# johndpope/SPEAK-hack

Hardware: NVIDIA B200
Metric: irfd_train_pairs_per_sec_256 (higher is better)
Workload: dtype bf16

## Files before the change

include/irfd_b200.h:

```cpp
#ifndef IRFD_B200_H_
#define IRFD_B200_H_

#include <stddef.h>
#include <stdint.h>

#ifdef __cplusplus
extern "C" {
#endif

#define IRFD_ABI_VERSION 1

#define IRFD_OK 0
#define IRFD_ERR_INVALID_ARGUMENT (-1)
#define IRFD_ERR_CUDA (-2)

typedef struct CUstream_st* irfd_stream_t;

int irfd_abi_version(void);
const char* irfd_last_error(void);

int irfd_conv_gemm_m_tiles(int n, int h, int w);
int irfd_conv_gemm_geometry(int n, int h, int w, int ksize, int wgroups, int* out_host);
int irfd_conv_gemm(const void* x, int n, int h, int w, int cin, const void* wk, int cout, int ksize, void* out,
                   void* out2, int mode, const float* bias, const float* nw, const float* noise, const float* sp1,
// ... 61 lines not shown
int irfd_conv_gemm_bnbwd_grouped(const void* x, int n, int h, int w, int cin, const void* wk, int cout, int ksize,
                                 void* out, const void* bn_z, const float* bn_mean, const float* bn_rstd,
                                 const float* const* bn_gamma, const float* const* bn_beta, float* partial,
                                 int stat_groups, int wgroups, int force_block_n, irfd_stream_t stream);
int irfd_conv_gemm_bnbwd_res_grouped(const void* x, int n, int h, int w, int cin, const void* wk, int cout, int ksize,
                                     void* out, const void* bn_z, const float* bn_mean, const float* bn_rstd,
                                     const void* g2, const void* mask_bits, float* partial, int stat_groups,
                                     int wgroups, int force_block_n, irfd_stream_t stream);
int irfd_bn_backward_finish_sets(const void* g, const void* z, const float* mean, const float* rstd,
                                 const float* const* gamma, void* dz, float* const* dgamma, float* const* dbeta,
                                 float grad_beta, int batch_stats, long long rows, int c, int groups, int nsets,
                                 const float* partial, int tiles, void* workspace, long long workspace_bytes,
                                 irfd_stream_t stream);

int irfd_pack_conv_weight(const float* w, void* dst, int o, int i, int taps, int mode, int kpad, irfd_stream_t stream);
int irfd_im2col_stem(const float* x, void* col, int n, int h, int w, int kpad, irfd_stream_t stream);
int irfd_im2col_3x3s2(const void* a, void* col, int n, int h, int w, int c, irfd_stream_t stream);
int irfd_col2im_3x3s2(const void* dcol, void* dx, int n, int h, int w, int c, irfd_stream_t stream);
int irfd_subsample2(const void* a, void* out, int n, int h, int w, int c, irfd_stream_t stream);
int irfd_scatter_add_s2(const void* a, const void* b, void* out, int n, int h, int w, int c, irfd_stream_t stream);
int irfd_maxpool_fwd(const void* a, void* out, void* argmax, int n, int h, int w, int c, irfd_stream_t stream);
int irfd_maxpool_bwd(const void* dout, const void* dout2, const void* argmax, void* dx, int n, int h, int w, int c,
                     irfd_stream_t stream);
int irfd_avgpool_fwd(const void* a, float* out, int n, int hw, int c, irfd_stream_t stream);
int irfd_avgpool_bwd(const float* dfeat, void* g, int n, int hw, int c, irfd_stream_t stream);
int irfd_nchw_to_nhwc_bf16(const float* in, void* out, int b, int c, int hw, int c_pad, irfd_stream_t stream);
int irfd_nhwc_bf16_to_nchw(const void* in, float* out, int b, int c, int hw, int c_pad, irfd_stream_t stream);

int irfd_const_input_fwd(const float* cst, const float* bias, const float* nw, const float* noise, const float* sp1,
                         const float* s1, void* a0, void* y0, int b, int c, irfd_stream_t stream);
int irfd_const_input_bwd(const void* dy, const void* a0, const float* noise, const float* sp1, float* dsp1, float* ds1,
                         float* dconst, float* dbias, float* dnw, int b, int c, irfd_stream_t stream);
int irfd_upsample2x_fwd(const void* in, void* out, int b, int h, int w, int c, irfd_stream_t stream);
int irfd_upsample2x_split_fwd(const void* in, const void* in_lo, void* out, int b, int h, int w, int c,
                              irfd_stream_t stream);
int irfd_const_input_split_fwd(const float* cst, const float* bias, const float* nw, const float* noise,
                               const float* sp1, const float* s1, void* a0, void* y0, void* y0_lo, int b, int c,
                               irfd_stream_t stream);
int irfd_upsample2x_bwd(const void* dout, void* din, int b, int h, int w, int c, irfd_stream_t stream);
int irfd_apply_noise_nchw(const float* x, const float* w, const float* noise, float* out, int b, int c, int hw,
                          irfd_stream_t stream);
int irfd_apply_style_nchw(const float* x, const float* style, float* out, int b, int c, int hw, irfd_stream_t stream);
long long irfd_style_bwd_workspace_bytes(int b, int hw, int c);
int irfd_style_bwd(const void* dy, const void* a, const float* noise, const float* sp1, void* dz, float* ds1,
                   float* dsp1, float* dbias, float* dnw, int b, int hw, int c, void* workspace,
                   long long workspace_bytes, irfd_stream_t stream);
// ... 49 lines not shown
```

speak_hack_b200/csrc/bn.cu:

```cuda
#include "host_util.h"
#include "rowvec.cuh"

namespace irfd {

constexpr int kMaxGroups = 4;
constexpr int kMaxSets = 4;
struct FSet {
  const float* p[kMaxSets];
};
struct FSetM {
  float* p[kMaxSets];
};
constexpr int kFinCh = 8;
constexpr int kFinLanes = 64;
constexpr int kFinThreads = kFinCh * kFinLanes;
constexpr int kFinWarps = kFinThreads / 32;
constexpr int kFinBatch = 8;

__device__ __forceinline__ void fin_partial_sums(const float* __restrict__ p0, const float* __restrict__ p1, size_t stride0,
                                                 size_t stride1, int n, int lane, double& a, double& b) {
  a = 0.0;
  b = 0.0;
  for (int t = lane; t < n; t += kFinLanes * kFinBatch) {
    float x[kFinBatch], y[kFinBatch];
#pragma unroll
    for (int u = 0; u < kFinBatch; ++u) {
      const int tt = t + u * kFinLanes;
      x[u] = tt < n ? __ldg(p0 + (size_t)tt * stride0) : 0.f;
      y[u] = tt < n ? __ldg(p1 + (size_t)tt * stride1) : 0.f;
    }
#pragma unroll
    for (int u = 0; u < kFinBatch; ++u) {
// ... 465 lines not shown
        L.g1, L.g2, L.act, L.z, L.mean, L.rstd, L.gamma, L.beta, L.partial, L.g_out, L.grows, L.c, L.rpb, L.gps,
        zigzag());
  else
    bn_bwd_reduce_kernel<HAS_G2, MASK, false><<<L.grid, kRvThreads, L.smem, L.stream>>>(
        L.g1, L.g2, L.act, L.z, L.mean, L.rstd, L.gamma, L.beta, L.partial, nullptr, L.grows, L.c, L.rpb, L.gps,
        zigzag());
  bn_bwd_finalize_kernel<<<dim3(L.c / kFinCh, L.nsets), kFinThreads, 0, L.stream>>>(L.partial, L.nblk, L.c, (double)L.grows,
                                                                             L.dgamma, L.dbeta, L.grad_beta, L.c1, L.c2,
                                                                             L.batch_stats, L.gps);
  if (L.g_out != nullptr)
    bn_bwd_apply_kernel<false, 0, false><<<L.grid, kRvThreads, 0, L.stream>>>(
        L.g_out, nullptr, nullptr, L.z, L.mean, L.rstd, L.gamma, L.beta, L.c1, L.c2, L.dz, nullptr, L.grows, L.c, L.rpb,
        L.gps);
  else
    bn_bwd_apply_kernel<HAS_G2, MASK, false><<<L.grid, kRvThreads, 0, L.stream>>>(
        L.g1, L.g2, L.act, L.z, L.mean, L.rstd, L.gamma, L.beta, L.c1, L.c2, L.dz, nullptr, L.grows, L.c, L.rpb,
        L.gps);
}

}

using namespace irfd;

static FSet make_fset(const float* const* ptrs, int nsets) {
  FSet f;
  for (int i = 0; i < kMaxSets; ++i) f.p[i] = (ptrs != nullptr && i < nsets) ? ptrs[i] : nullptr;
  return f;
}
static FSetM make_fsetm(float* const* ptrs, int nsets) {
  FSetM f;
  for (int i = 0; i < kMaxSets; ++i) f.p[i] = (ptrs != nullptr && i < nsets) ? ptrs[i] : nullptr;
  return f;
}

extern "C" int irfd_bn_finalize_sets(const float* psum, const float* psq, int tiles, int c, long long count, float eps,
                                     float momentum, float* mean, float* rstd, float* const* running_mean,
                                     float* const* running_var, int running_updates, int groups, int nsets,
                                     cudaStream_t stream) {
  IRFD_CHECK_ARG(psum && psq && mean && rstd && tiles > 0 && c > 0 && count > 0, "bn_finalize: bad argument");
  IRFD_CHECK_ARG(groups >= 1 && groups <= kMaxGroups, "bn_finalize: 1..4 statistic groups per set");
  IRFD_CHECK_ARG(nsets >= 1 && nsets <= kMaxSets, "bn_finalize: 1..4 parameter sets");
  IRFD_CHECK_ARG(c % kFinCh == 0, "bn_finalize: C must be a multiple of 8 (got %d)", c);
  IRFD_CHECK_ARG((running_mean == nullptr) == (running_var == nullptr), "bn_finalize: running buffers come in pairs");
  bn_finalize_kernel<<<dim3(c / kFinCh, nsets), kFinThreads, 0, stream>>>(psum, psq, tiles, c, (double)count, eps, momentum,
                                                                     mean, rstd, make_fsetm(running_mean, nsets),
                                                                     make_fsetm(running_var, nsets), running_updates,
                                                                     groups);
  IRFD_CHECK_LAUNCH();
  return IRFD_OK;
}

// ... 198 lines not shown
```

speak_hack_b200/csrc/layout.cu:

```cuda
#include "host_util.h"
#include "rowvec.cuh"

namespace irfd {

__global__ void pack_weight_kernel(const float* __restrict__ w, __nv_bfloat16* __restrict__ dst, int O, int I, int T,
                                   int mode, int kpad) {
  const size_t idx = (size_t)blockIdx.x * blockDim.x + threadIdx.x;
  if (mode == 3) {
    if (idx >= (size_t)O * kpad) return;
    const int o = idx / kpad, k = idx % kpad;
    dst[idx] = __float2bfloat16(k < I * T ? w[(size_t)o * I * T + k] : 0.f);
    return;
  }
  if (idx >= (size_t)O * I * T) return;
  const int tap = idx % T;
  const int i = (idx / T) % I;
  const int o = idx / ((size_t)T * I);
  const __nv_bfloat16 v = __float2bfloat16(w[idx]);
  size_t d;
  if (mode == 0) d = ((size_t)o * T + tap) * I + i;
  else if (mode == 1) d = ((size_t)i * T + (T - 1 - tap)) * O + o;
  else d = ((size_t)tap * I + i) * O + o;
  dst[d] = v;
}
// ... 44 lines not shown
#pragma unroll
    for (int t = 0; t < 8; ++t) f[t] = off[t] >= 0 ? srow[off[t] + 2 * ow] : 0.f;
    store8(col + (pix0 + ow) * kpad + v * 8, f);
  }
}

__global__ void im2col_3x3s2_kernel(const __nv_bfloat16* __restrict__ a, __nv_bfloat16* __restrict__ col, int N, int H,
                                    int W, int C) {
  const unsigned Ho = (H + 1) / 2, Wo = (W + 1) / 2, vc = C / 8;
  const unsigned idx = blockIdx.x * blockDim.x + threadIdx.x;
  const size_t total = (size_t)N * Ho * Wo * 9 * vc;
  if (idx >= total) return;
  const int v = idx % vc;
  const int tap = (idx / vc) % 9;
  const unsigned pix = idx / (vc * 9u);
  const int ow = pix % Wo, oh = (pix / Wo) % Ho, n = pix / ((unsigned)Wo * Ho);
  const int ih = oh * 2 + tap / 3 - 1, iw = ow * 2 + tap % 3 - 1;
  uint4 val = make_uint4(0, 0, 0, 0);
  if (ih >= 0 && ih < H && iw >= 0 && iw < W)
    val = *reinterpret_cast<const uint4*>(a + (((size_t)n * H + ih) * W + iw) * C + v * 8);
  *reinterpret_cast<uint4*>(col + ((size_t)pix * 9 + tap) * C + v * 8) = val;
}

__global__ void col2im_3x3s2_kernel(const __nv_bfloat16* __restrict__ dcol, __nv_bfloat16* __restrict__ dx, int N,
                                    int H, int W, int C) {
  const unsigned Ho = H / 2, Wo = W / 2, vc = C / 8;
  const unsigned idx = blockIdx.x * blockDim.x + threadIdx.x;
  const size_t total = (size_t)N * H * W * vc;
  if (idx >= total) return;
  const int v = idx % vc;
  const unsigned pix = idx / vc;
  const int w = pix % W, h = (pix / W) % H, n = pix / ((unsigned)W * H);
  float acc[8];
#pragma unroll
  for (int t = 0; t < 8; ++t) acc[t] = 0.f;
  for (int kh = 0; kh < 3; ++kh) {
    const int th = h - kh + 1;
    if (th < 0 || (th & 1)) continue;
    const int oh = th >> 1;
    if (oh >= Ho) continue;
    for (int kw = 0; kw < 3; ++kw) {
      const int tw = w - kw + 1;
      if (tw < 0 || (tw & 1)) continue;
      const int ow = tw >> 1;
      if (ow >= Wo) continue;
      float f[8];
// ... 20 lines not shown
__global__ void scatter_add_s2_kernel(const __nv_bfloat16* __restrict__ a, const __nv_bfloat16* __restrict__ b,
                                      __nv_bfloat16* __restrict__ out, int N, int H, int W, int C) {
  const unsigned vc = C / 8;
  const unsigned idx = blockIdx.x * blockDim.x + threadIdx.x;
  if (idx >= (size_t)N * H * W * vc) return;
  const int v = idx % vc;
  const unsigned pix = idx / vc;
  const int w = pix % W, h = (pix / W) % H, n = pix / ((unsigned)W * H);
  float f[8];
  if (a != nullptr) load8(a + (size_t)pix * C + v * 8, f);
  else {
#pragma unroll
    for (int t = 0; t < 8; ++t) f[t] = 0.f;
  }
  if (!(h & 1) && !(w & 1)) {
    float g[8];
    load8(b + (((size_t)n * (H / 2) + h / 2) * (W / 2) + w / 2) * C + v * 8, g);
#pragma unroll
    for (int t = 0; t < 8; ++t) f[t] += g[t];
  }
  store8(out + (size_t)pix * C + v * 8, f);
}

__global__ void maxpool_fwd_kernel(const __nv_bfloat16* __restrict__ a, __nv_bfloat16* __restrict__ out,
                                   uint8_t* __restrict__ arg, int N, int H, int W, int C) {
  const unsigned Ho = (H + 1) / 2, Wo = (W + 1) / 2, vc = C / 8;
  const unsigned idx = blockIdx.x * blockDim.x + threadIdx.x;
  if (idx >= (size_t)N * Ho * Wo * vc) return;
  const int v = idx % vc;
  const unsigned pix = idx / vc;
  const int ow = pix % Wo, oh = (pix / Wo) % Ho, n = pix / ((unsigned)Wo * Ho);
  float best[8];
  int bi[8];
#pragma unroll
  for (int t = 0; t < 8; ++t) {
    best[t] = -INFINITY;
    bi[t] = 0;
  }
  for (int tap = 0; tap < 9; ++tap) {
    const int ih = oh * 2 + tap / 3 - 1, iw = ow * 2 + tap % 3 - 1;
    if (ih < 0 || ih >= H || iw < 0 || iw >= W) continue;
    float f[8];
    load8(a + (((size_t)n * H + ih) * W + iw) * C + v * 8, f);
#pragma unroll
    for (int t = 0; t < 8; ++t)
      if (f[t] > best[t]) {
        best[t] = f[t];
        bi[t] = tap;
      }
  }
  store8(out + (size_t)pix * C + v * 8, best);
  uint2 packed;
  packed.x = bi[0] | (bi[1] << 8) | (bi[2] << 16) | (bi[3] << 24);
  packed.y = bi[4] | (bi[5] << 8) | (bi[6] << 16) | (bi[7] << 24);
  *reinterpret_cast<uint2*>(arg + (size_t)pix * C + v * 8) = packed;
}

__global__ void __launch_bounds__(256)
maxpool_bwd_kernel(const __nv_bfloat16* __restrict__ dout, const __nv_bfloat16* __restrict__ dout2,
                   const uint8_t* __restrict__ arg, __nv_bfloat16* __restrict__ dx, int N, int H, int W, int C) {
  const unsigned Ho = H / 2, Wo = W / 2, vc = C >> 3;
  const unsigned q = blockIdx.y * blockDim.x + threadIdx.x;
  if (q >= Wo * vc) return;
  const int j = q / vc, v = q - j * vc;
  const int n = blockIdx.x / Ho, i = blockIdx.x - n * Ho;
  float g[2][2][8];
  uint2 am[2][2];
#pragma unroll
  for (int a = 0; a < 2; ++a)
#pragma unroll
    for (int b = 0; b < 2; ++b) {
      am[a][b] = make_uint2(0xffffffffu, 0xffffffffu);
#pragma unroll
      for (int t = 0; t < 8; ++t) g[a][b][t] = 0.f;
      if ((unsigned)(i + a) < Ho && (unsigned)(j + b) < Wo) {
        const size_t op = (((size_t)n * Ho + i + a) * Wo + j + b) * C + v * 8;
        am[a][b] = __ldg(reinterpret_cast<const uint2*>(arg + op));
        unpack8(ldg16(dout + op), g[a][b]);
// ... 119 lines not shown
  return IRFD_OK;
}

extern "C" int irfd_im2col_stem(const float* x, void* col, int n, int h, int w, int kpad, cudaStream_t stream) {
  IRFD_CHECK_ARG(x && col && kpad >= 152 && kpad % 8 == 0 && h > 0 && w > 0, "im2col_stem: bad argument");
  const size_t smem = (size_t)21 * (w + 6) * sizeof(float);
  IRFD_CHECK_ARG(n > 0 && smem <= 48 * 1024, "im2col_stem: image too wide for the row stage (W <= 579, got %d)", w);
  IRFD_CHECK_ARG(kStemPixPar * (kpad / 8) <= 256 && (kpad / 8) % 4 == 0, "im2col_stem: kpad a multiple of 32 and <= 256");
  im2col_stem_kernel<<<(unsigned)(n * ((h + 1) / 2)), kStemPixPar * (kpad / 8), smem, stream>>>(x, BF(col), n, h, w,
                                                                                              kpad);
  IRFD_CHECK_LAUNCH();
  return IRFD_OK;
}

extern "C" int irfd_im2col_3x3s2(const void* a, void* col, int n, int h, int w, int c, cudaStream_t stream) {
  IRFD_CHECK_ARG(a && col && c % 8 == 0 && h > 0 && w > 0, "im2col_3x3s2: bad argument");
  const size_t total = (size_t)n * ((h + 1) / 2) * ((w + 1) / 2) * 9 * (c / 8);
  CHECK_TOTAL32(total);
  im2col_3x3s2_kernel<<<GRID1D(total)>>>(CBF(a), BF(col), n, h, w, c);
  IRFD_CHECK_LAUNCH();
  return IRFD_OK;
}

extern "C" int irfd_col2im_3x3s2(const void* dcol, void* dx, int n, int h, int w, int c, cudaStream_t stream) {
  IRFD_CHECK_ARG(dcol && dx && c % 8 == 0 && h % 2 == 0 && w % 2 == 0, "col2im_3x3s2: bad argument");
  const size_t total = (size_t)n * h * w * (c / 8);
  CHECK_TOTAL32(total);
  col2im_3x3s2_kernel<<<GRID1D(total)>>>(CBF(dcol), BF(dx), n, h, w, c);
  IRFD_CHECK_LAUNCH();
  return IRFD_OK;
}

extern "C" int irfd_subsample2(const void* a, void* out, int n, int h, int w, int c, cudaStream_t stream) {
  IRFD_CHECK_ARG(a && out && c % 8 == 0 && h > 0 && w > 0, "subsample2: bad argument");
  const size_t total = (size_t)n * ((h + 1) / 2) * ((w + 1) / 2) * (c / 8);
  CHECK_TOTAL32(total);
  subsample2_kernel<<<GRID1D(total)>>>(CBF(a), BF(out), n, h, w, c);
  IRFD_CHECK_LAUNCH();
  return IRFD_OK;
}

extern "C" int irfd_scatter_add_s2(const void* a, const void* b, void* out, int n, int h, int w, int c,
                                   cudaStream_t stream) {
  IRFD_CHECK_ARG(b && out && c % 8 == 0 && h % 2 == 0 && w % 2 == 0, "scatter_add_s2: bad argument");
  const size_t total = (size_t)n * h * w * (c / 8);
  CHECK_TOTAL32(total);
  scatter_add_s2_kernel<<<GRID1D(total)>>>(CBF(a), CBF(b), BF(out), n, h, w, c);
  IRFD_CHECK_LAUNCH();
  return IRFD_OK;
}

extern "C" int irfd_maxpool_fwd(const void* a, void* out, void* argmax, int n, int h, int w, int c,
                                cudaStream_t stream) {
  IRFD_CHECK_ARG(a && out && argmax && c % 8 == 0 && h > 0 && w > 0, "maxpool_fwd: bad argument");
  const size_t total = (size_t)n * ((h + 1) / 2) * ((w + 1) / 2) * (c / 8);
  CHECK_TOTAL32(total);
  maxpool_fwd_kernel<<<GRID1D(total)>>>(CBF(a), BF(out), reinterpret_cast<uint8_t*>(argmax), n, h, w, c);
  IRFD_CHECK_LAUNCH();
  return IRFD_OK;
}

extern "C" int irfd_maxpool_bwd(const void* dout, const void* dout2, const void* argmax, void* dx, int n, int h, int w,
                                int c, cudaStream_t stream) {
  IRFD_CHECK_ARG(dout && dx && argmax && c % 8 == 0 && h % 2 == 0 && w % 2 == 0, "maxpool_bwd: bad argument");
  IRFD_CHECK_ARG((long long)w * c < (1ll << 24) && (long long)n * h < (1ll << 31), "maxpool_bwd: bad shape");
  maxpool_bwd_kernel<<<dim3((unsigned)(n * (h / 2)), (unsigned)(((w / 2) * (c / 8) + 255) / 256)), 256, 0, stream>>>(
      CBF(dout), CBF(dout2), reinterpret_cast<const uint8_t*>(argmax), BF(dx), n, h, w, c);
  IRFD_CHECK_LAUNCH();
  return IRFD_OK;
}

extern "C" int irfd_avgpool_fwd(const void* a, float* out, int n, int hw, int c, cudaStream_t stream) {
  IRFD_CHECK_ARG(a && out && c % 8 == 0 && c <= 2048 && hw > 0, "avgpool_fwd: bad argument");
  avgpool_fwd_kernel<<<n, kRvThreads, 2048 * sizeof(float), stream>>>(CBF(a), out, hw, c);
  IRFD_CHECK_LAUNCH();
  return IRFD_OK;
}

extern "C" int irfd_avgpool_bwd(const float* dfeat, void* g, int n, int hw, int c, cudaStream_t stream) {
  IRFD_CHECK_ARG(dfeat && g && c % 8 == 0 && hw > 0, "avgpool_bwd: bad argument");
// ... 23 lines not shown
```

speak_hack_b200/csrc/rowvec.cuh:

```cuda
#pragma once
#include <stdlib.h>
#include "ptx.cuh"

namespace irfd {

constexpr int kRvThreads = 256;

struct RowVec {
  int cv;
  int row_lane;
  int rows_par;
  bool active;
  __device__ RowVec(int C) {
    const int vec_per_row = C >> 3;
    rows_par = kRvThreads / vec_per_row;
    if (rows_par < 1) rows_par = 1;
    cv = threadIdx.x % vec_per_row;
    row_lane = threadIdx.x / vec_per_row;
    active = row_lane < rows_par;
  }
};

constexpr int kRowBatch = 4;

__device__ __forceinline__ uint4 ldg16(const __nv_bfloat16* p) { return __ldg(reinterpret_cast<const uint4*>(p)); }
__device__ __forceinline__ void unpack8(const uint4& u, float (&f)[8]) {
  float2 a = unpack_bf16x2(u.x), b = unpack_bf16x2(u.y), c = unpack_bf16x2(u.z), d = unpack_bf16x2(u.w);
  f[0] = a.x; f[1] = a.y; f[2] = b.x; f[3] = b.y; f[4] = c.x; f[5] = c.y; f[6] = d.x; f[7] = d.y;
}
__device__ __forceinline__ void load8(const __nv_bfloat16* p, float (&f)[8]) {
  const uint4 u = *reinterpret_cast<const uint4*>(p);
  unpack8(u, f);
}
__device__ __forceinline__ void store8(__nv_bfloat16* p, const float (&f)[8]) {
  uint4 u;
  u.x = pack_bf16x2(f[0], f[1]);
  u.y = pack_bf16x2(f[2], f[3]);
  u.z = pack_bf16x2(f[4], f[5]);
  u.w = pack_bf16x2(f[6], f[7]);
  *reinterpret_cast<uint4*>(p) = u;
}
__device__ __forceinline__ void loadf8(const float* p, float (&f)[8]) {
  const float4 a = *reinterpret_cast<const float4*>(p);
  const float4 b = *reinterpret_cast<const float4*>(p + 4);
  f[0] = a.x; f[1] = a.y; f[2] = a.z; f[3] = a.w; f[4] = b.x; f[5] = b.y; f[6] = b.z; f[7] = b.w;
}

template <int K>
__device__ __forceinline__ void block_reduce_rows(const RowVec& rv, int C, float (&acc)[K][8], float* smem, float* dst,
                                                  size_t dst_stride) {
  if (rv.active) {
#pragma unroll
    for (int k = 0; k < K; ++k)
#pragma unroll
      for (int t = 0; t < 8; ++t) smem[((size_t)k * rv.rows_par + rv.row_lane) * C + rv.cv * 8 + t] = acc[k][t];
  }
  __syncthreads();
  if (rv.active && rv.row_lane == 0) {
#pragma unroll
    for (int k = 0; k < K; ++k)
#pragma unroll
      for (int t = 0; t < 8; ++t) {
        float s = 0.f;
        for (int l = 0; l < rv.rows_par; ++l) s += smem[((size_t)k * rv.rows_par + l) * C + rv.cv * 8 + t];
        dst[k * dst_stride + rv.cv * 8 + t] = s;
      }
  }
}

inline int row_block_waves() {
// ... 21 lines not shown
```

speak_hack_b200/encoder_group.py:

```python
from __future__ import annotations

import os
from typing import Dict, List, Optional

import torch
import torch.nn as nn

from . import ops
from .encoder import BN_EPS, BN_MOMENTUM, MAX_STEM_W, MIN_HW, ResNet50Encoder, trainable_shape


fold_bn_reduce = os.environ.get("IRFD_BN_FOLD", "1") != "0"
fold_bn3_reduce = os.environ.get("IRFD_BN3_FOLD", "0") != "0"


def _stack_pack(convs, mode, kpad=0):
    return ops.pack_conv_weights_stacked([c.weight for c in convs], mode, kpad)


class _Stats:
    __slots__ = ("mean", "rstd")

    def __init__(self, mean, rstd):
        self.mean, self.rstd = mean, rstd


def _group_inference(grp: "EncoderGroup", x, col0=None):
    encs = grp.encoders
    E = len(encs)
    x = x.contiguous().to(torch.float32)
    n, _, h, w = x.shape
    if col0 is None:
        col0 = ops.im2col_stem(x, 192)
    sc, sh = ops.bn_eval_affine_sets([e[1] for e in encs])
    a0 = ops.conv_gemm_affine_grouped(col0, _stack_pack([e[0] for e in encs], ops.PACK_FLAT, 192), 1, sc, sh, relu=True,
                                      wgroups=E, a_shared=True).view(E * n, ops.half_up(h), ops.half_up(w), 64)
# ... 28 lines not shown


class _EncoderGroupFn(torch.autograd.Function):

    @staticmethod
    def forward(ctx, x, grp, stat_groups, col0, recorded, *params):
        encs: List[ResNet50Encoder] = grp.encoders
        E = len(encs)
        G = stat_groups
        GT = E * G
        U = 2 if (recorded and all(getattr(e, "_recompute_bn_update", False) for e in encs)) else 1
        x = x.contiguous().to(torch.float32)
        n, _, h, w = x.shape

        def stats(bns, s, q, rows_total):
            mean, rstd = ops.bn_finalize_sets(s, q, rows_total // GT, BN_EPS, BN_MOMENTUM,
                                              [b.running_mean for b in bns], [b.running_var for b in bns], U, G, E)
            return _Stats(mean, rstd)

        def apply(z, st, bns, relu=True, res=None, bn2=None, want_mask=False):
            return ops.bn_apply_sets(z, st.mean, st.rstd, [b.weight for b in bns], [b.bias for b in bns], res=res,
                                     bn2=bn2, relu=relu, groups=GT, want_mask=want_mask)

        S = {}
        if col0 is None:
            col0 = ops.im2col_stem(x, 192)
        bn0 = [e[1] for e in encs]
        z0, s, q = ops.conv_gemm_grouped(col0, _stack_pack([e[0] for e in encs], ops.PACK_FLAT, 192), 1, ops.EPI_STATS,
                                         wgroups=E, a_shared=True)
        h1, w1 = h // 2, w // 2
        z0 = z0.view(E * n, h1, w1, 64)
        st0 = stats(bn0, s, q, E * n * h1 * w1)
        a0 = apply(z0, st0, bn0)
        cur, arg0 = ops.maxpool_fwd(a0)
        S["stem"] = (col0, z0, st0, a0, arg0)
        S["blocks"] = []
        for li in range(4, 8):
            for bi in range(len(encs[0][li])):
                blks = [e[li][bi] for e in encs]
                xin = cur
                nb, hh, ww, _cin = xin.shape
                z1, s, q = ops.conv_gemm_grouped(xin, _stack_pack([b.conv1 for b in blks], ops.PACK_FPROP), 1,
                                                 ops.EPI_STATS, wgroups=E)
                bn1 = [b.bn1 for b in blks]
                st1 = stats(bn1, s, q, nb * hh * ww)
                a1 = apply(z1, st1, bn1)
                planes = a1.shape[-1]
                wk2 = _stack_pack([b.conv2 for b in blks], ops.PACK_FPROP)
                col2 = None
                if blks[0].stride == 1:
                    z2, s, q = ops.conv_gemm_grouped(a1, wk2, 3, ops.EPI_STATS, wgroups=E)
                    ho, wo = hh, ww
                else:
                    col2 = ops.im2col_3x3s2(a1)
                    ho, wo = hh // 2, ww // 2
                    z2, s, q = ops.conv_gemm_grouped(col2.view(1, 1, col2.shape[0], 9 * planes), wk2, 1, ops.EPI_STATS,
                                                     wgroups=E)
                    z2 = z2.view(nb, ho, wo, planes)
                bn2 = [b.bn2 for b in blks]
                st2 = stats(bn2, s, q, nb * ho * wo)
                a2 = apply(z2, st2, bn2)
                z3, s, q = ops.conv_gemm_grouped(a2, _stack_pack([b.conv3 for b in blks], ops.PACK_FPROP), 1,
                                                 ops.EPI_STATS, wgroups=E)
                bn3 = [b.bn3 for b in blks]
                st3 = stats(bn3, s, q, nb * ho * wo)
                xs = zd = std = None
                if blks[0].downsample is not None:
                    xs = ops.subsample2(xin) if blks[0].stride == 2 else xin
                    zd, s, q = ops.conv_gemm_grouped(xs, _stack_pack([b.downsample[0] for b in blks], ops.PACK_FPROP), 1,
                                                     ops.EPI_STATS, wgroups=E)
                    dbn = [b.downsample[1] for b in blks]
                    std = stats(dbn, s, q, nb * ho * wo)
                    out = apply(z3, st3, bn3, res=zd, want_mask=recorded,
                                bn2=(std.mean, std.rstd, [b.weight for b in dbn], [b.bias for b in dbn]))
                else:
                    out = apply(z3, st3, bn3, res=xin, want_mask=recorded)
                out, obits = out if recorded else (out, None)
# ... 42 lines not shown
                d_a = ops.conv_gemm_grouped(dy, wk, ksize, wgroups=E)
                return lambda: bn_bwd(bns, st, d_a, None, None, z, mask_from_z=True)
            gm, part = ops.conv_gemm_bnbwd_grouped(dy, wk, ksize, z, st.mean, st.rstd, [b.weight for b in bns],
                                                   [b.bias for b in bns], GT)
            return lambda: ops.bn_backward_finish_sets(gm, z, st.mean, st.rstd, [b.weight for b in bns], part,
                                                       dgammas=[tgt(b.weight) for b in bns],
                                                       dbetas=[tgt(b.bias) for b in bns], groups=GT)[0]

        side = ops.side_stream(dfeat.device)

        def wgrad(convs, xx, dy, ksize, **kw):
            dws = [tgt(c.weight) for c in convs]
            side.launch(lambda: ops.conv_wgrad_grouped(xx, dy, ksize, dws, **kw), xx, dy, *dws)

        cur_li = None
        pre = None
        blocks = S["blocks"]
        for bidx in range(len(blocks) - 1, -1, -1):
            li, blks, xin, z1, st1, a1, col2, z2, st2, a2, z3, st3, xs, zd, std, obits = blocks[bidx]
            if cur_li is not None and li != cur_li and cb is not None:
                cb("stage", cur_li)
            cur_li = li
            nb, hh, ww, _cin = xin.shape
            planes = a1.shape[-1]
            if pre is not None:
                gmask, part3 = pre
                bn3 = [b.bn3 for b in blks]
                dz3 = ops.bn_backward_finish_sets(gmask, z3, st3.mean, st3.rstd, [b.weight for b in bn3], part3,
                                                  dgammas=[tgt(b.weight) for b in bn3],
                                                  dbetas=[tgt(b.bias) for b in bn3], groups=GT)[0]
                pre = None
            else:
                dz3, gmask = bn_bwd([b.bn3 for b in blks], st3, g, g2, None, z3, want_g_out=True, act_bits=obits)
            finish = dgrad_bn(dz3, [b.conv3 for b in blks], 1, [b.bn2 for b in blks], st2, z2)
            wgrad([b.conv3 for b in blks], a2, dz3, 1)
            dz2 = finish()
            if blks[0].stride == 1:
                finish = dgrad_bn(dz2, [b.conv2 for b in blks], 3, [b.bn1 for b in blks], st1, z1)
                wgrad([b.conv2 for b in blks], a1, dz2, 3)
                dz1 = finish()
            else:
                m2 = dz2.numel() // planes
                dcol = ops.conv_gemm_grouped(dz2.view(1, 1, m2, planes),
                                             _stack_pack([b.conv2 for b in blks], ops.PACK_DCOL), 1, wgroups=E)
                wgrad([b.conv2 for b in blks], col2, dz2.view(m2, planes), 1, reduce_cin=planes, reduce_taps=9)
                d_a1 = ops.col2im_3x3s2(dcol.view(m2, 9 * planes), nb, hh, ww, planes)
                dz1 = bn_bwd([b.bn1 for b in blks], st1, d_a1, None, a1, z1, mask_from_z=True)
            wk1 = _stack_pack([b.conv1 for b in blks], ops.PACK_DGRAD)
            if blks[0].downsample is None and fold_bn3_reduce:
                prev = blocks[bidx - 1]
                pre = ops.conv_gemm_bnbwd_res_grouped(dz1, wk1, 1, prev[10], prev[11].mean, prev[11].rstd, gmask,
                                                      prev[15], GT, wgroups=E)
                wgrad([b.conv1 for b in blks], xin, dz1, 1)
                continue
            d_in = ops.conv_gemm_grouped(dz1, wk1, 1, wgroups=E)
            wgrad([b.conv1 for b in blks], xin, dz1, 1)
            if blks[0].downsample is not None:
                dzd = bn_bwd([b.downsample[1] for b in blks], std, gmask, None, None, zd)
                d_xs = ops.conv_gemm_grouped(dzd, _stack_pack([b.downsample[0] for b in blks], ops.PACK_DGRAD), 1,
                                             wgroups=E)
                wgrad([b.downsample[0] for b in blks], xs, dzd, 1)
                if blks[0].stride == 2:
                    g, g2 = ops.scatter_add_s2(d_in, d_xs), None
                else:
                    g, g2 = d_in, d_xs
            else:
                g, g2 = d_in, gmask
        if cb is not None and cur_li is not None:
            cb("stage", cur_li)
        col0, z0, st0, a0, arg0 = S["stem"]
        d_a0 = ops.maxpool_bwd(g, arg0, g2)
        dz0 = bn_bwd([e[1] for e in encs], st0, d_a0, None, a0, z0, mask_from_z=True)
        wgrad([e[0] for e in encs], col0, dz0.view(-1, 64), 1, x_shared=True, reduce_cin=147, reduce_taps=1)
        side.join()
        if cb is not None:
            cb("stage", 3)
            cb("post", None)
        ctx.S = None
        if targets is not None:
            return (None,) * (5 + sum(len(e._flat_params()) for e in encs))
        return (None, None, None, None, None) + tuple(grads.get(p) for e in encs for p in e._flat_params())


class EncoderGroup:

    def __init__(self, encoders: List[ResNet50Encoder]):
        self.encoders = list(encoders)
        self.grad_targets: Optional[Dict[nn.Parameter, torch.Tensor]] = None
        self._bwd_cb = None

    def can_run(self, x: torch.Tensor, groups: int) -> bool:
        encs = self.encoders
        if not (x.is_cuda and x.dim() == 4 and x.shape[1] == 3 and x.size(0) % groups == 0):
            return False
        if len({e.training for e in encs}) != 1:
# ... 28 lines not shown
```

speak_hack_b200/ops.py:

```python
from __future__ import annotations

import ctypes
import os
import weakref
from typing import Optional

import torch

from . import _lib

BF16 = torch.bfloat16
F32 = torch.float32

EPI_PLAIN, EPI_STATS, EPI_STYLE = 0, 1, 2
PACK_FPROP, PACK_DGRAD, PACK_DCOL, PACK_FLAT = 0, 1, 2, 3

launch_count = 0


def _stream() -> int:
    return torch.cuda.current_stream().cuda_stream


def _ptr(t: Optional[torch.Tensor]) -> Optional[int]:
# ... 495 lines not shown
    rstd = torch.empty((tot, c), dtype=F32, device=ssum.device)
    _call("irfd_bn_finalize_sets", ssum.data_ptr(), ssq.data_ptr(), tiles // tot, c, int(count), eps, momentum,
          mean.data_ptr(), rstd.data_ptr(), _ptr_array(running_means), _ptr_array(running_vars), running_updates, groups,
          nsets, _stream())
    return mean, rstd


def bn_apply_sets(z, mean, rstd, gammas, betas, res=None, bn2=None, relu=True, groups=1, want_mask=False):
    _chk(z, BF16, "z")
    c = z.shape[-1]
    rows = z.numel() // c
    out = torch.empty_like(z)
    bits = torch.empty((rows, c // 8), dtype=torch.uint8, device=z.device) if want_mask else None
    m2 = r2 = g2 = b2 = None
    if bn2 is not None:
        m2, r2, g2, b2 = bn2
    _call("irfd_bn_apply_sets", z.data_ptr(), mean.data_ptr(), rstd.data_ptr(), _ptr_array(gammas), _ptr_array(betas),
          _ptr(res), _ptr(m2), _ptr(r2), _ptr_array(g2) if g2 is not None else _ptr_array([None] * len(gammas)),
          _ptr_array(b2) if b2 is not None else _ptr_array([None] * len(gammas)), out.data_ptr(), _ptr(bits), rows, c,
          1 if relu else 0, groups, len(gammas), _stream())
    return (out, bits) if want_mask else out


def _bn_bwd_bytes(rows, c, has_g2, mask_units, want_g_out):
    n_in = 2 + (1 if has_g2 else 0) + mask_units
    if want_g_out:
        return 2.0 * rows * c * (n_in + 1 + 3)
    return 2.0 * rows * c * (2 * n_in + 1)


def bn_backward_sets(g1, g2, act, z, mean, rstd, gammas, betas=None, dgammas=None, dbetas=None, want_g_out=False,
                     batch_stats=True, groups=1, act_bits=None):
    lib = _lib.load()
    c = z.shape[-1]
    rows = z.numel() // c
    nsets = len(gammas)
    dz = torch.empty_like(z)
    g_out = torch.empty_like(z) if want_g_out else None
    if dgammas is None:
        dg_all = torch.empty((nsets, c), dtype=F32, device=z.device)
        db_all = torch.empty((nsets, c), dtype=F32, device=z.device)
        dgammas, dbetas = list(dg_all.unbind(0)), list(db_all.unbind(0))
    ws = workspace(lib.irfd_bn_bwd_workspace_bytes(rows, c, groups), z.device)
    if act_bits is not None and act is not None:
        raise _lib.IrfdError("bn_backward_sets: pass act or act_bits, not both")
    mask_units = 1.0 if act is not None else (1.0 / 16 if act_bits is not None else 0.0)
# ... 37 lines not shown


def half_up(x: int) -> int:
    return (x + 1) // 2


def resnet_stage_hw(h: int, w: int):
    sizes = [(half_up(h), half_up(w))]
    for _ in range(4):
        sizes.append((half_up(sizes[-1][0]), half_up(sizes[-1][1])))
    return sizes


def im2col_stem(x: torch.Tensor, kpad: int = 192) -> torch.Tensor:
    _chk(x, F32, "x")
    n, c, h, w = x.shape
    if c != 3:
        raise _lib.IrfdError("im2col_stem expects 3 input channels")
    col = torch.empty((n * half_up(h) * half_up(w), kpad), dtype=BF16, device=x.device)
    _call("irfd_im2col_stem", x.data_ptr(), col.data_ptr(), n, h, w, kpad, _stream())
    return col


def im2col_3x3s2(a: torch.Tensor) -> torch.Tensor:
    n, h, w, c = a.shape
    col = torch.empty((n * half_up(h) * half_up(w), 9 * c), dtype=BF16, device=a.device)
    _call("irfd_im2col_3x3s2", a.data_ptr(), col.data_ptr(), n, h, w, c, _stream())
    return col


def col2im_3x3s2(dcol: torch.Tensor, n, h, w, c) -> torch.Tensor:
    dx = torch.empty((n, h, w, c), dtype=BF16, device=dcol.device)
    _call("irfd_col2im_3x3s2", dcol.data_ptr(), dx.data_ptr(), n, h, w, c, _stream())
    return dx


def subsample2(a: torch.Tensor) -> torch.Tensor:
    n, h, w, c = a.shape
    out = torch.empty((n, half_up(h), half_up(w), c), dtype=BF16, device=a.device)
    _call("irfd_subsample2", a.data_ptr(), out.data_ptr(), n, h, w, c, _stream())
    return out


def scatter_add_s2(a: Optional[torch.Tensor], b: torch.Tensor) -> torch.Tensor:
    n, h2, w2, c = b.shape
    out = torch.empty((n, h2 * 2, w2 * 2, c), dtype=BF16, device=b.device)
    _call("irfd_scatter_add_s2", _ptr(a), b.data_ptr(), out.data_ptr(), n, h2 * 2, w2 * 2, c, _stream())
    return out


def maxpool_fwd(a: torch.Tensor):
    n, h, w, c = a.shape
    out = torch.empty((n, half_up(h), half_up(w), c), dtype=BF16, device=a.device)
    arg = torch.empty((n, half_up(h), half_up(w), c), dtype=torch.uint8, device=a.device)
    _call("irfd_maxpool_fwd", a.data_ptr(), out.data_ptr(), arg.data_ptr(), n, h, w, c, _stream())
    return out, arg


def maxpool_bwd(dout: torch.Tensor, arg: torch.Tensor, dout2: Optional[torch.Tensor] = None) -> torch.Tensor:
    n, h2, w2, c = dout.shape
    dx = torch.empty((n, h2 * 2, w2 * 2, c), dtype=BF16, device=dout.device)
    _call("irfd_maxpool_bwd", dout.data_ptr(), _ptr(dout2), arg.data_ptr(), dx.data_ptr(), n, h2 * 2, w2 * 2, c,
          _stream())
    return dx


def avgpool_fwd(a: torch.Tensor) -> torch.Tensor:
    n, h, w, c = a.shape
    out = torch.empty((n, c), dtype=F32, device=a.device)
    _call("irfd_avgpool_fwd", a.data_ptr(), out.data_ptr(), n, h * w, c, _stream())
    return out


def avgpool_bwd(dfeat: torch.Tensor, h: int, w: int) -> torch.Tensor:
    _chk(dfeat, F32, "dfeat")
    n, c = dfeat.shape
    g = torch.empty((n, h, w, c), dtype=BF16, device=dfeat.device)
    _call("irfd_avgpool_bwd", dfeat.data_ptr(), g.data_ptr(), n, h * w, c, _stream())
# ... 290 lines not shown
```

Measured before the change: 889.4.

## Fold BN+ReLU apply into stem maxpool and stride-2 im2col in encoder forward

```diff
diff --git a/include/irfd_b200.h b/include/irfd_b200.h
--- a/include/irfd_b200.h
+++ b/include/irfd_b200.h
@@ -107,6 +107,12 @@
 int irfd_maxpool_fwd(const void* a, void* out, void* argmax, int n, int h, int w, int c, irfd_stream_t stream);
 int irfd_maxpool_bwd(const void* dout, const void* dout2, const void* argmax, void* dx, int n, int h, int w, int c,
                      irfd_stream_t stream);
+int irfd_im2col_3x3s2_bnrelu(const void* z, const float* mean, const float* rstd, const float* const* gamma,
+                             const float* const* beta, void* col, int n, int h, int w, int c, int groups, int nsets,
+                             irfd_stream_t stream);
+int irfd_maxpool_fwd_bnrelu(const void* z, const float* mean, const float* rstd, const float* const* gamma,
+                            const float* const* beta, void* out, void* argmax, int n, int h, int w, int c, int groups,
+                            int nsets, irfd_stream_t stream);
 int irfd_avgpool_fwd(const void* a, float* out, int n, int hw, int c, irfd_stream_t stream);
 int irfd_avgpool_bwd(const float* dfeat, void* g, int n, int hw, int c, irfd_stream_t stream);
 int irfd_nchw_to_nhwc_bf16(const float* in, void* out, int b, int c, int hw, int c_pad, irfd_stream_t stream);
diff --git a/speak_hack_b200/csrc/bn.cu b/speak_hack_b200/csrc/bn.cu
--- a/speak_hack_b200/csrc/bn.cu
+++ b/speak_hack_b200/csrc/bn.cu
@@ -4,10 +4,6 @@
 namespace irfd {
 
 constexpr int kMaxGroups = 4;
-constexpr int kMaxSets = 4;
-struct FSet {
-  const float* p[kMaxSets];
-};
 struct FSetM {
   float* p[kMaxSets];
 };
@@ -519,11 +515,6 @@
 
 using namespace irfd;
 
-static FSet make_fset(const float* const* ptrs, int nsets) {
-  FSet f;
-  for (int i = 0; i < kMaxSets; ++i) f.p[i] = (ptrs != nullptr && i < nsets) ? ptrs[i] : nullptr;
-  return f;
-}
 static FSetM make_fsetm(float* const* ptrs, int nsets) {
   FSetM f;
   for (int i = 0; i < kMaxSets; ++i) f.p[i] = (ptrs != nullptr && i < nsets) ? ptrs[i] : nullptr;
diff --git a/speak_hack_b200/csrc/layout.cu b/speak_hack_b200/csrc/layout.cu
--- a/speak_hack_b200/csrc/layout.cu
+++ b/speak_hack_b200/csrc/layout.cu
@@ -90,6 +90,26 @@
   *reinterpret_cast<uint4*>(col + ((size_t)pix * 9 + tap) * C + v * 8) = val;
 }
 
+__global__ void im2col_3x3s2_bnrelu_kernel(const __nv_bfloat16* __restrict__ z, BnRelu bn, __nv_bfloat16* __restrict__ col,
+                                           int N, int H, int W, int C) {
+  const unsigned Ho = (H + 1) / 2, Wo = (W + 1) / 2, vc = C / 8;
+  const unsigned idx = blockIdx.x * blockDim.x + threadIdx.x;
+  if (idx >= (size_t)N * Ho * Wo * vc) return;
+  const int v = idx % vc;
+  const unsigned pix = idx / vc;
+  const int ow = pix % Wo, oh = (pix / Wo) % Ho, n = pix / ((unsigned)Wo * Ho);
+  float sc[8], sh[8];
+  bn_relu_coeffs(bn, n, C, v * 8, sc, sh);
+#pragma unroll
+  for (int tap = 0; tap < 9; ++tap) {
+    const int ih = oh * 2 + tap / 3 - 1, iw = ow * 2 + tap % 3 - 1;
+    uint4 val = make_uint4(0, 0, 0, 0);
+    if (ih >= 0 && ih < H && iw >= 0 && iw < W)
+      val = bn_relu8(ldg16(z + (((size_t)n * H + ih) * W + iw) * C + v * 8), sc, sh);
+    *reinterpret_cast<uint4*>(col + ((size_t)pix * 9 + tap) * C + v * 8) = val;
+  }
+}
+
 __global__ void col2im_3x3s2_kernel(const __nv_bfloat16* __restrict__ dcol, __nv_bfloat16* __restrict__ dx, int N,
                                     int H, int W, int C) {
   const unsigned Ho = H / 2, Wo = W / 2, vc = C / 8;
@@ -156,38 +176,67 @@
   store8(out + (size_t)pix * C + v * 8, f);
 }
 
-__global__ void maxpool_fwd_kernel(const __nv_bfloat16* __restrict__ a, __nv_bfloat16* __restrict__ out,
-                                   uint8_t* __restrict__ arg, int N, int H, int W, int C) {
-  const unsigned Ho = (H + 1) / 2, Wo = (W + 1) / 2, vc = C / 8;
-  const unsigned idx = blockIdx.x * blockDim.x + threadIdx.x;
-  if (idx >= (size_t)N * Ho * Wo * vc) return;
-  const int v = idx % vc;
-  const unsigned pix = idx / vc;
-  const int ow = pix % Wo, oh = (pix / Wo) % Ho, n = pix / ((unsigned)Wo * Ho);
-  float best[8];
-  int bi[8];
-#pragma unroll
-  for (int t = 0; t < 8; ++t) {
-    best[t] = -INFINITY;
-    bi[t] = 0;
-  }
-  for (int tap = 0; tap < 9; ++tap) {
-    const int ih = oh * 2 + tap / 3 - 1, iw = ow * 2 + tap % 3 - 1;
-    if (ih < 0 || ih >= H || iw < 0 || iw >= W) continue;
-    float f[8];
-    load8(a + (((size_t)n * H + ih) * W + iw) * C + v * 8, f);
-#pragma unroll
-    for (int t = 0; t < 8; ++t)
-      if (f[t] > best[t]) {
-        best[t] = f[t];
-        bi[t] = tap;
-      }
-  }
-  store8(out + (size_t)pix * C + v * 8, best);
-  uint2 packed;
-  packed.x = bi[0] | (bi[1] << 8) | (bi[2] << 16) | (bi[3] << 24);
-  packed.y = bi[4] | (bi[5] << 8) | (bi[6] << 16) | (bi[7] << 24);
-  *reinterpret_cast<uint2*>(arg + (size_t)pix * C + v * 8) = packed;
+template <bool BN>
+__global__ void __launch_bounds__(256)
+maxpool_fwd_kernel(const __nv_bfloat16* __restrict__ a, BnRelu bn, __nv_bfloat16* __restrict__ out,
+                   uint8_t* __restrict__ arg, int N, int H, int W, int C) {
+  const unsigned Ho = (H + 1) / 2, Wo = (W + 1) / 2, Wp = (Wo + 1) / 2, vc = C / 8;
+  const unsigned idx = blockIdx.x * blockDim.x + threadIdx.x;
+  if (idx >= (size_t)N * Ho * Wp * vc) return;
+  const int v = idx % vc;
+  const unsigned pp = idx / vc;
+  const int j = pp % Wp, oh = (pp / Wp) % Ho, n = pp / ((unsigned)Wp * Ho);
+  uint4 q[3][5];
+#pragma unroll
+  for (int kh = 0; kh < 3; ++kh) {
+    const int ih = oh * 2 + kh - 1;
+#pragma unroll
+    for (int k = 0; k < 5; ++k) {
+      const int iw = j * 4 + k - 1;
+      q[kh][k] = make_uint4(0, 0, 0, 0);
+      if (ih >= 0 && ih < H && iw >= 0 && iw < W) q[kh][k] = ldg16(a + (((size_t)n * H + ih) * W + iw) * C + v * 8);
+    }
+  }
+  if (BN) {
+    float sc[8], sh[8];
+    bn_relu_coeffs(bn, n, C, v * 8, sc, sh);
+#pragma unroll
+    for (int kh = 0; kh < 3; ++kh)
+#pragma unroll
+      for (int k = 0; k < 5; ++k) q[kh][k] = bn_relu8(q[kh][k], sc, sh);
+  }
+#pragma unroll
+  for (int o = 0; o < 2; ++o) {
+    const int ow = j * 2 + o;
+    if (ow >= (int)Wo) break;
+    float best[8];
+    int bi[8];
+#pragma unroll
+    for (int t = 0; t < 8; ++t) {
+      best[t] = -INFINITY;
+      bi[t] = 0;
+    }
+#pragma unroll
+    for (int tap = 0; tap < 9; ++tap) {
+      const int kh = tap / 3, kw = tap % 3;
+      const int ih = oh * 2 + kh - 1, iw = ow * 2 + kw - 1;
+      if (ih < 0 || ih >= H || iw < 0 || iw >= W) continue;
+      float f[8];
+      unpack8(q[kh][o * 2 + kw], f);
+#pragma unroll
+      for (int t = 0; t < 8; ++t)
+        if (f[t] > best[t]) {
+          best[t] = f[t];
+          bi[t] = tap;
+        }
+    }
+    const size_t pix = ((size_t)n * Ho + oh) * Wo + ow;
+    store8(out + pix * C + v * 8, best);
+    uint2 packed;
+    packed.x = bi[0] | (bi[1] << 8) | (bi[2] << 16) | (bi[3] << 24);
+    packed.y = bi[4] | (bi[5] << 8) | (bi[6] << 16) | (bi[7] << 24);
+    *reinterpret_cast<uint2*>(arg + pix * C + v * 8) = packed;
+  }
 }
 
 __global__ void __launch_bounds__(256)
@@ -353,6 +402,32 @@
   return IRFD_OK;
 }
 
+static int make_bn_relu(const float* mean, const float* rstd, const float* const* gamma, const float* const* beta, int n,
+                        int h, int w, int groups, int nsets, BnRelu* bn) {
+  IRFD_CHECK_ARG(mean && rstd && gamma && beta, "bn_relu: null BatchNorm pointer");
+  IRFD_CHECK_ARG(nsets >= 1 && nsets <= kMaxSets, "bn_relu: 1..4 parameter sets");
+  IRFD_CHECK_ARG(groups >= 1 && groups % nsets == 0 && n % groups == 0,
+                 "bn_relu: %d images must split evenly into %d groups of %d sets", n, groups, nsets);
+  for (int s = 0; s < nsets; ++s) IRFD_CHECK_ARG(gamma[s] && beta[s], "bn_relu: null gamma/beta of set %d", s);
+  *bn = BnRelu{mean, rstd, make_fset(gamma, nsets), make_fset(beta, nsets), n / groups,
+               groups / nsets};
+  return IRFD_OK;
+}
+
+extern "C" int irfd_im2col_3x3s2_bnrelu(const void* z, const float* mean, const float* rstd, const float* const* gamma,
+                                        const float* const* beta, void* col, int n, int h, int w, int c, int groups,
+                                        int nsets, cudaStream_t stream) {
+  IRFD_CHECK_ARG(z && col && c % 8 == 0 && n > 0 && h > 0 && w > 0, "im2col_3x3s2_bnrelu: bad argument");
+  BnRelu bn;
+  const int rc = make_bn_relu(mean, rstd, gamma, beta, n, h, w, groups, nsets, &bn);
+  if (rc != IRFD_OK) return rc;
+  const size_t total = (size_t)n * ((h + 1) / 2) * ((w + 1) / 2) * (c / 8);
+  CHECK_TOTAL32(total * 9);
+  im2col_3x3s2_bnrelu_kernel<<<GRID1D(total)>>>(CBF(z), bn, BF(col), n, h, w, c);
+  IRFD_CHECK_LAUNCH();
+  return IRFD_OK;
+}
+
 extern "C" int irfd_col2im_3x3s2(const void* dcol, void* dx, int n, int h, int w, int c, cudaStream_t stream) {
   IRFD_CHECK_ARG(dcol && dx && c % 8 == 0 && h % 2 == 0 && w % 2 == 0, "col2im_3x3s2: bad argument");
   const size_t total = (size_t)n * h * w * (c / 8);
@@ -384,9 +459,24 @@
 extern "C" int irfd_maxpool_fwd(const void* a, void* out, void* argmax, int n, int h, int w, int c,
                                 cudaStream_t stream) {
   IRFD_CHECK_ARG(a && out && argmax && c % 8 == 0 && h > 0 && w > 0, "maxpool_fwd: bad argument");
-  const size_t total = (size_t)n * ((h + 1) / 2) * ((w + 1) / 2) * (c / 8);
-  CHECK_TOTAL32(total);
-  maxpool_fwd_kernel<<<GRID1D(total)>>>(CBF(a), BF(out), reinterpret_cast<uint8_t*>(argmax), n, h, w, c);
+  const size_t total = (size_t)n * ((h + 1) / 2) * (((w + 1) / 2 + 1) / 2) * (c / 8);
+  CHECK_TOTAL32(total);
+  maxpool_fwd_kernel<false><<<GRID1D(total)>>>(CBF(a), BnRelu{}, BF(out), reinterpret_cast<uint8_t*>(argmax), n, h, w,
+                                                c);
+  IRFD_CHECK_LAUNCH();
+  return IRFD_OK;
+}
+
+extern "C" int irfd_maxpool_fwd_bnrelu(const void* z, const float* mean, const float* rstd, const float* const* gamma,
+                                       const float* const* beta, void* out, void* argmax, int n, int h, int w, int c,
+                                       int groups, int nsets, cudaStream_t stream) {
+  IRFD_CHECK_ARG(z && out && argmax && c % 8 == 0 && n > 0 && h > 0 && w > 0, "maxpool_fwd_bnrelu: bad argument");
+  BnRelu bn;
+  const int rc = make_bn_relu(mean, rstd, gamma, beta, n, h, w, groups, nsets, &bn);
+  if (rc != IRFD_OK) return rc;
+  const size_t total = (size_t)n * ((h + 1) / 2) * (((w + 1) / 2 + 1) / 2) * (c / 8);
+  CHECK_TOTAL32(total);
+  maxpool_fwd_kernel<true><<<GRID1D(total)>>>(CBF(z), bn, BF(out), reinterpret_cast<uint8_t*>(argmax), n, h, w, c);
   IRFD_CHECK_LAUNCH();
   return IRFD_OK;
 }
diff --git a/speak_hack_b200/csrc/rowvec.cuh b/speak_hack_b200/csrc/rowvec.cuh
--- a/speak_hack_b200/csrc/rowvec.cuh
+++ b/speak_hack_b200/csrc/rowvec.cuh
@@ -46,6 +46,58 @@
   f[0] = a.x; f[1] = a.y; f[2] = a.z; f[3] = a.w; f[4] = b.x; f[5] = b.y; f[6] = b.z; f[7] = b.w;
 }
 
+constexpr int kMaxSets = 4;
+struct FSet {
+  const float* p[kMaxSets];
+};
+inline FSet make_fset(const float* const* ptrs, int nsets) {
+  FSet f;
+  for (int i = 0; i < kMaxSets; ++i) f.p[i] = (ptrs != nullptr && i < nsets) ? ptrs[i] : nullptr;
+  return f;
+}
+
+struct BnRelu {
+  const float* mean;
+  const float* rstd;
+  FSet gamma, beta;
+  int group_imgs;
+  int gps;
+};
+__device__ __forceinline__ void bn_relu_coeffs(const BnRelu& p, int n, int C, int c0, float (&sc)[8], float (&sh)[8]) {
+  const int g = n / p.group_imgs;
+  const int set = g / p.gps;
+  const float* gamma = p.gamma.p[0];
+  const float* beta = p.beta.p[0];
+#pragma unroll
+  for (int s = 1; s < kMaxSets; ++s)
+    if (s == set) {
+      gamma = p.gamma.p[s];
+      beta = p.beta.p[s];
+    }
+  float m[8], r[8], ga[8], be[8];
+  loadf8(p.mean + (size_t)g * C + c0, m);
+  loadf8(p.rstd + (size_t)g * C + c0, r);
+  loadf8(gamma + c0, ga);
+  loadf8(beta + c0, be);
+#pragma unroll
+  for (int t = 0; t < 8; ++t) {
+    sc[t] = ga[t] * r[t];
+    sh[t] = be[t] - m[t] * sc[t];
+  }
+}
+__device__ __forceinline__ uint4 bn_relu8(const uint4& q, const float (&sc)[8], const float (&sh)[8]) {
+  float v[8], o[8];
+  unpack8(q, v);
+#pragma unroll
+  for (int t = 0; t < 8; ++t) o[t] = fmaxf(v[t] * sc[t] + sh[t], 0.f);
+  uint4 u;
+  u.x = pack_bf16x2(o[0], o[1]);
+  u.y = pack_bf16x2(o[2], o[3]);
+  u.z = pack_bf16x2(o[4], o[5]);
+  u.w = pack_bf16x2(o[6], o[7]);
+  return u;
+}
+
 template <int K>
 __device__ __forceinline__ void block_reduce_rows(const RowVec& rv, int C, float (&acc)[K][8], float* smem, float* dst,
                                                   size_t dst_stride) {
diff --git a/speak_hack_b200/encoder_group.py b/speak_hack_b200/encoder_group.py
--- a/speak_hack_b200/encoder_group.py
+++ b/speak_hack_b200/encoder_group.py
@@ -12,6 +12,7 @@
 
 fold_bn_reduce = os.environ.get("IRFD_BN_FOLD", "1") != "0"
 fold_bn3_reduce = os.environ.get("IRFD_BN3_FOLD", "0") != "0"
+fold_bn_apply = os.environ.get("IRFD_BN_APPLY_FOLD", "1") != "0"
 
 
 def _stack_pack(convs, mode, kpad=0):
@@ -86,6 +87,9 @@
             return ops.bn_apply_sets(z, st.mean, st.rstd, [b.weight for b in bns], [b.bias for b in bns], res=res,
                                      bn2=bn2, relu=relu, groups=GT, want_mask=want_mask)
 
+        def bn_relu(st, bns):
+            return st.mean, st.rstd, [b.weight for b in bns], [b.bias for b in bns], GT
+
         S = {}
         if col0 is None:
             col0 = ops.im2col_stem(x, 192)
@@ -95,9 +99,11 @@
         h1, w1 = h // 2, w // 2
         z0 = z0.view(E * n, h1, w1, 64)
         st0 = stats(bn0, s, q, E * n * h1 * w1)
-        a0 = apply(z0, st0, bn0)
-        cur, arg0 = ops.maxpool_fwd(a0)
-        S["stem"] = (col0, z0, st0, a0, arg0)
+        if fold_bn_apply:
+            cur, arg0 = ops.maxpool_fwd(z0, bn=bn_relu(st0, bn0))
+        else:
+            cur, arg0 = ops.maxpool_fwd(apply(z0, st0, bn0))
+        S["stem"] = (col0, z0, st0, arg0)
         S["blocks"] = []
         for li in range(4, 8):
             for bi in range(len(encs[0][li])):
@@ -108,15 +114,16 @@
                                                  ops.EPI_STATS, wgroups=E)
                 bn1 = [b.bn1 for b in blks]
                 st1 = stats(bn1, s, q, nb * hh * ww)
-                a1 = apply(z1, st1, bn1)
-                planes = a1.shape[-1]
+                planes = z1.shape[-1]
                 wk2 = _stack_pack([b.conv2 for b in blks], ops.PACK_FPROP)
-                col2 = None
+                a1 = col2 = None
                 if blks[0].stride == 1:
+                    a1 = apply(z1, st1, bn1)
                     z2, s, q = ops.conv_gemm_grouped(a1, wk2, 3, ops.EPI_STATS, wgroups=E)
                     ho, wo = hh, ww
                 else:
-                    col2 = ops.im2col_3x3s2(a1)
+                    col2 = (ops.im2col_3x3s2(z1, bn=bn_relu(st1, bn1)) if fold_bn_apply
+                            else ops.im2col_3x3s2(apply(z1, st1, bn1)))
                     ho, wo = hh // 2, ww // 2
                     z2, s, q = ops.conv_gemm_grouped(col2.view(1, 1, col2.shape[0], 9 * planes), wk2, 1, ops.EPI_STATS,
                                                      wgroups=E)
@@ -205,7 +212,7 @@
                 cb("stage", cur_li)
             cur_li = li
             nb, hh, ww, _cin = xin.shape
-            planes = a1.shape[-1]
+            planes = z1.shape[-1]
             if pre is not None:
                 gmask, part3 = pre
                 bn3 = [b.bn3 for b in blks]
@@ -228,7 +235,7 @@
                                              _stack_pack([b.conv2 for b in blks], ops.PACK_DCOL), 1, wgroups=E)
                 wgrad([b.conv2 for b in blks], col2, dz2.view(m2, planes), 1, reduce_cin=planes, reduce_taps=9)
                 d_a1 = ops.col2im_3x3s2(dcol.view(m2, 9 * planes), nb, hh, ww, planes)
-                dz1 = bn_bwd([b.bn1 for b in blks], st1, d_a1, None, a1, z1, mask_from_z=True)
+                dz1 = bn_bwd([b.bn1 for b in blks], st1, d_a1, None, None, z1, mask_from_z=True)
             wk1 = _stack_pack([b.conv1 for b in blks], ops.PACK_DGRAD)
             if blks[0].downsample is None and fold_bn3_reduce:
                 prev = blocks[bidx - 1]
@@ -251,9 +258,9 @@
                 g, g2 = d_in, gmask
         if cb is not None and cur_li is not None:
             cb("stage", cur_li)
-        col0, z0, st0, a0, arg0 = S["stem"]
+        col0, z0, st0, arg0 = S["stem"]
         d_a0 = ops.maxpool_bwd(g, arg0, g2)
-        dz0 = bn_bwd([e[1] for e in encs], st0, d_a0, None, a0, z0, mask_from_z=True)
+        dz0 = bn_bwd([e[1] for e in encs], st0, d_a0, None, None, z0, mask_from_z=True)
         wgrad([e[0] for e in encs], col0, dz0.view(-1, 64), 1, x_shared=True, reduce_cin=147, reduce_taps=1)
         side.join()
         if cb is not None:
diff --git a/speak_hack_b200/ops.py b/speak_hack_b200/ops.py
--- a/speak_hack_b200/ops.py
+++ b/speak_hack_b200/ops.py
@@ -541,6 +541,12 @@
     return (out, bits) if want_mask else out
 
 
+def bn_relu_args(c, mean, rstd, gammas, betas, groups):
+    if mean.shape != rstd.shape or tuple(mean.shape) != (groups, c) or len(gammas) != len(betas):
+        raise _lib.IrfdError("bn_relu: mean/rstd must be [groups, C] and gammas/betas one per set")
+    return mean.data_ptr(), rstd.data_ptr(), _ptr_array(gammas), _ptr_array(betas)
+
+
 def _bn_bwd_bytes(rows, c, has_g2, mask_units, want_g_out):
     n_in = 2 + (1 if has_g2 else 0) + mask_units
     if want_g_out:
@@ -624,10 +630,15 @@
     return col
 
 
-def im2col_3x3s2(a: torch.Tensor) -> torch.Tensor:
+def im2col_3x3s2(a: torch.Tensor, bn=None) -> torch.Tensor:
     n, h, w, c = a.shape
     col = torch.empty((n * half_up(h) * half_up(w), 9 * c), dtype=BF16, device=a.device)
-    _call("irfd_im2col_3x3s2", a.data_ptr(), col.data_ptr(), n, h, w, c, _stream())
+    if bn is None:
+        _call("irfd_im2col_3x3s2", a.data_ptr(), col.data_ptr(), n, h, w, c, _stream())
+    else:
+        _chk(a, BF16, "z")
+        _call("irfd_im2col_3x3s2_bnrelu", a.data_ptr(), *bn_relu_args(c, *bn), col.data_ptr(), n, h, w, c, bn[4],
+              len(bn[2]), _stream())
     return col
 
 
@@ -651,11 +662,16 @@
     return out
 
 
-def maxpool_fwd(a: torch.Tensor):
+def maxpool_fwd(a: torch.Tensor, bn=None):
     n, h, w, c = a.shape
     out = torch.empty((n, half_up(h), half_up(w), c), dtype=BF16, device=a.device)
     arg = torch.empty((n, half_up(h), half_up(w), c), dtype=torch.uint8, device=a.device)
-    _call("irfd_maxpool_fwd", a.data_ptr(), out.data_ptr(), arg.data_ptr(), n, h, w, c, _stream())
+    if bn is None:
+        _call("irfd_maxpool_fwd", a.data_ptr(), out.data_ptr(), arg.data_ptr(), n, h, w, c, _stream())
+    else:
+        _chk(a, BF16, "z")
+        _call("irfd_maxpool_fwd_bnrelu", a.data_ptr(), *bn_relu_args(c, *bn), out.data_ptr(), arg.data_ptr(), n, h, w, c,
+              bn[4], len(bn[2]), _stream())
     return out, arg
 
 
```

After: 897.8 (median of 6 runs). Within noise of the previous version (+0.9%).
